# visinf/veto

Hardware: AMD Instinct MI355X
Metric: relation-pairs/sec (PredCls, 36 obj/img) (higher is better)
Workload: dtype fp16 + e4m3 correction terms (fp16 MFMA main product, e4m3 K=128 MFMA cross terms, fp32 accumulate); 1 GPU; BASELINE.json configs[1]: synthetic PredCls, 12 img x 36 obj = 15120 pairs/GPU, d=576, 8 heads, 4 layers, 51 predicates; images_per_gpu=12, objects_per_image=36, pairs_per_gpu=15120, layers=4, heads=8, precision=mixed, parallelism=single GPU

## Files before the change

### veto_amd/csrc/abi_forward.hip

```cpp
#include "abi_internal.h"

namespace {

struct Workspace {
  int32_t *subj, *obj;
  float* lc;
  __bf16* pa;
  float* patch_tab;
  float* x;
  __bf16* a;
  char* big;
  float* xc;
  __bf16* ptab_split;
  float *sw, *ow;
  float* stats;
  __bf16 *ac, *hc;
  size_t total;
};

Workspace carve(char* base, int n_obj, int n_pair, int chunk) {
  Workspace w;
  size_t off = 0;
  auto take = [&](size_t bytes) {
    char* ptr = base ? base + off : nullptr;
    off += align_up(bytes, 256);
    return ptr;
  };
  const size_t prow = (size_t)gemm_rows_padded(n_obj * 16);
  const size_t tile_rows = qkv_attn_rows_padded(chunk);
  const size_t mpad = (size_t)gemm_rows_padded((int)(tile_rows > (size_t)chunk * kTokens ? tile_rows : (size_t)chunk * kTokens));
  const size_t cpad = (size_t)gemm_rows_padded(chunk);
  w.subj = (int32_t*)take((size_t)n_pair * 4);
  w.obj = (int32_t*)take((size_t)n_pair * 4);
  w.lc = (float*)take((size_t)n_obj * 2 * 2 * kDim * 4);
  w.pa = (__bf16*)take(prow * 2 * 2048 * 2);
  w.patch_tab = (float*)take((size_t)n_obj * 16 * 2 * kDim * 4);
  w.x = (float*)take(mpad * kDim * 4);
  w.a = (__bf16*)take(mpad * 2 * kDim * 2);
  {
    const size_t qkv_bytes = mpad * 3 * kDim * 4, fold_bytes = 2 * (align_up(cpad * (size_t)cls_fold_max_heads() * kDim * 4, 256));
    w.big = take(qkv_bytes > fold_bytes ? qkv_bytes : fold_bytes);
  }
  w.xc = (float*)take(cpad * kDim * 4);
  w.ptab_split = (__bf16*)take(prow * 2 * 2 * kDim * 2);
  w.sw = (float*)take(prow * 3 * kDim * 4);
  w.ow = (float*)take(prow * 3 * kDim * 4);
  w.stats = (float*)take(mpad * 2 * 4);
  w.ac = (__bf16*)take(cpad * 2 * kDim * 2);
  w.hc = (__bf16*)take(cpad * 4 * kDim * 2);
  w.total = off;
  return w;
}

struct ForwardPlan {
  int L, H, dhp;
  bool qkv0_tables, fold_last, mixed, fast, mixed_out, cls_mixed, tail_fused, panel, qkv_f24, qa_fused, x_f24;
  bool ffn_ln_next(int l) const { return mixed && panel && l + 1 < L - 1; }
};

ForwardPlan make_plan(veto_handle_t h, bool sat) {
  ForwardPlan p;
  const int L = p.L = h->cfg.layers, H = p.H = h->cfg.heads;
  p.dhp = h->fold_dhp;
  static const bool tables_off = env_knob_is("VETO_QKV0_TABLES", "0");
  p.qkv0_tables = L >= 2 && !tables_off;
  static const bool fold_off = env_knob_is("VETO_CLS_FOLD", "0");
  p.fold_last = !fold_off && H <= cls_fold_max_heads();
  p.mixed = h->cfg.precision != VETO_PRECISE;
  p.fast = h->cfg.precision == VETO_FAST;
  p.mixed_out = p.mixed && attention_reads_tables(H);
  p.cls_mixed = p.mixed;
  static const bool tail_off = env_knob_is("VETO_TAIL_FUSED", "0");
  p.tail_fused = !tail_off && !sat;
  p.panel = !sat;
  static const bool qkv_f24_off = env_knob_is("VETO_QKV_F24", "0");
  p.qkv_f24 = !qkv_f24_off && attention_reads_tables(H);
  static const bool qa_off = env_knob_is("VETO_QKV_ATTN_FUSED", "0");
  p.qa_fused = p.mixed && p.mixed_out && p.tail_fused && !qa_off && qkv_attn_fused_supports(H);
  static const bool x_f24_on = env_knob_is("VETO_X_F24", "1");
  p.x_f24 = x_f24_on && !p.fast && p.mixed && p.mixed_out && p.tail_fused && p.fold_last && p.qkv0_tables && p.qa_fused && L >= 3;
  return p;
}

int object_side(veto_handle_t h, hipStream_t s, const Workspace& ws, const ForwardPlan& p, const veto_inputs_t* in,
                const veto_debug_outputs_t* dbg) {
  const int n_obj = in->n_obj, n_pair = in->n_pair;
  {
    ProfScope ps(h, s, "pair_indices", 0, (double)n_pair * 24);
    HIP_TRY(launch_pair_indices(in->rel_pairs, in->img_obj_offset, in->img_pair_offset, in->n_img, n_pair, ws.subj,
                                ws.obj, dbg ? dbg->subj_inds : nullptr, dbg ? dbg->obj_inds : nullptr, s));
  }
  {
    if (in->bn_batch_stats) HIP_TRY(launch_bn_batch_stats(in->boxes, in->box_mode, n_obj, in->bn_batch_stats, s));
    const ObjPrepArgs a = obj_prep_args(h, in, ws.lc);
    ProfScope ps(h, s, "obj_prep", 2.0 * n_obj * 2 * kDim * (kPosDim + h->cfg.embed_dim), (double)n_obj * 2 * 2 * kDim * 4);
    HIP_TRY(launch_obj_prep(a, s));
  }
  {
// ... 44 lines not shown
    return VETO_OK;
  }

  int qkv0_from_tables() {
    const LayerW& w = h->layers[0];
    const bool mixed = p.mixed;
    if (!attention_reads_tables(p.H)) {
      ProfScope ps(h, s, "qkv0_combine", 0, (double)np * 17 * 3 * kDim * 4 * 3);
      HIP_TRY(launch_qkv0_combine(ws.sw, ws.ow, ws.stats, h->q0_vec, ws.subj + c0, ws.obj + c0, qkv(), np, s));
    }
    for (int t = kTokens - 2; t < kTokens; ++t) {
      if (mixed) HIP_TRY(count_sat(0, VETO_SAT_QKV_IN, ws.a + (size_t)t * 2 * kDim, (long)kTokens * kDim * 4, np, kDim));
      int rc = run_gemm(h, s, "gemm_qkv0_lc", ws.a + (size_t)t * 2 * kDim, mixed ? w.qkv_m : w.qkv, nullptr, nullptr, 0,
                        qkv() + (size_t)t * 3 * kDim, nullptr, (long)kTokens * 3 * kDim, np, 3 * kDim, kDim, EPI_F32, (long)kTokens * 2 * kDim, 0,
                        DropSite(), mixed ? w.exp_m + LIN_QKV : nullptr);
      if (rc) return rc;
    }
    return VETO_OK;
  }

  int attention(int l, bool qkv_f24) {
    const bool last = l == p.L - 1;
    AttnArgs a{};
    a.qkv = qkv(); a.n_pair = np; a.heads = p.H; a.cls_only = last ? 1 : 0;
    a.qkv_f24 = qkv_f24 ? 1 : 0;
    a.o = last ? ws.ac : ws.a;
    a.o_fmt = (!last && p.mixed_out) ? FMT_MIXED : FMT_SPLIT;
    if (l == 0 && p.qkv0_tables && attention_reads_tables(p.H)) {
      a.sw = ws.sw; a.ow = ws.ow; a.stats = ws.stats; a.vec = h->q0_vec; a.subj = ws.subj + c0; a.obj = ws.obj + c0;
    }
    const double nq = last ? 1 : kTokens;
    ProfScope ps(h, s, last ? "attention_cls" : "attention", 4.0 * np * nq * kTokens * kDim,
                 (double)M * 3 * kDim * (qkv_f24 ? 3 : 4) + (double)np * nq * kDim * 4);
    HIP_TRY(launch_attention(a, s));
    if (a.o_fmt == FMT_MIXED) HIP_TRY(count_sat(l, VETO_SAT_ATTN_OUT, ws.a, (long)kDim * 4, M, kDim));
    return VETO_OK;
  }

  int qkv_attention(int l, bool* attn_in_big) {
    const LayerW& w = h->layers[l];
    if (p.qa_fused && l > 0) {
      QkvAttnArgs q{};
      q.a = (const char*)ws.a; q.w = (const char*)w.qkv_m; q.w_exp = w.exp_m + LIN_QKV; q.o = ws.big; q.n_pair = np; q.heads = p.H; q.fast = p.fast ? 1 : 0;
      ProfScope ps(h, s, "qkv_attn_fused", 2.0 * M * 3.0 * kDim * kDim + 4.0 * np * kTokens * kTokens * kDim,
                   (double)M * kDim * 8 + 3.0 * kDim * kDim * 4);
      HIP_TRY(launch_qkv_attn_fused(q, s));
      *attn_in_big = true;
      return VETO_OK;
    }
    const bool mq = p.mixed && l > 0;
    const bool qkv_f24 = mq && p.qkv_f24;
    if (mq) HIP_TRY(count_sat(l, VETO_SAT_QKV_IN, ws.a, (long)kDim * 4, M, kDim));
    int rc = run_gemm(h, s, "gemm_qkv", ws.a, mq ? w.qkv_m : w.qkv, nullptr, nullptr, 0, qkv(), nullptr, 3 * kDim, M, 3 * kDim, kDim,
                      qkv_f24 ? EPI_F24 : EPI_F32, 0, 0, DropSite(), mq ? w.exp_m + LIN_QKV : nullptr);
    return rc ? rc : attention(l, qkv_f24);
  }

  int layer_tail_one_launch(int l, bool attn_in_big) {
    const LayerW& w = h->layers[l];
    const LayerW& nx = h->layers[l + 1];
    const bool ln_next = p.ffn_ln_next(l);
    char* rows = attn_in_big ? ws.big : (char*)ws.a;
    const RowNorm next{ln_next ? nx.ln1_w : nullptr, ln_next ? nx.ln1_b : nullptr, attn_in_big ? ws.a : nullptr};
    FfnArgs f = layer_tail_args(rows, w.mixed(LIN_OUT), RowNorm{w.ln2_w, w.ln2_b, rows}, w.mixed(LIN_FC1), w.mixed(LIN_FC2), ws.x, M, next);
    f.fast = p.fast ? 1 : 0;
    if (p.x_f24) {
// ... 236 lines not shown
```

### veto_amd/csrc/attention.hip

```cpp
#include "common.h"
#include "kernels.h"

#include <cstdio>
#include <cstdlib>
#include <cstring>

namespace veto {

namespace {

constexpr int kWavesPerBlock = 4;

__global__ __launch_bounds__(256) void attention_kernel(AttnArgs a, int dh, int ldh ) {
  extern __shared__ __attribute__((aligned(16))) char smem_raw[];
  const int lane = threadIdx.x & 63, w = threadIdx.x >> 6;
  const long gw = (long)blockIdx.x * kWavesPerBlock + w;
  const int per_wave = 3 * kTokens * ldh + kTokens * 20;
  float* sq = (float*)smem_raw + (size_t)w * per_wave;
  float* sk = sq + kTokens * ldh;
  float* sv = sk + kTokens * ldh;
  float* sp = sv + kTokens * ldh;
  const bool active = gw < (long)a.n_pair * a.heads;
  const int pair = active ? (int)(gw / a.heads) : 0;
  const int head = active ? (int)(gw % a.heads) : 0;
// ... 62 lines not shown
__device__ __forceinline__ void att_split2(float a, float b, uint32_t& hi, uint32_t& lo) {
  uint32_t h, l;
  float l0, l1;
  asm volatile("v_cvt_pk_f16_f32 %0, %1, %2" : "=v"(h) : "v"(a), "v"(b));
  asm("v_fma_mix_f32 %0, %1, -1.0, %2 op_sel_hi:[1,0,0]" : "=v"(l0) : "v"(h), "v"(a));
  asm("v_fma_mix_f32 %0, %1, -1.0, %2 op_sel:[1,0,0] op_sel_hi:[1,0,0]" : "=v"(l1) : "v"(h), "v"(b));
  asm volatile("v_cvt_pk_f16_f32 %0, %1, %2" : "=v"(l) : "v"(l0), "v"(l1));
  hi = h;
  lo = l;
}
typedef _Float16 att_f16x8 __attribute__((ext_vector_type(8)));
__device__ __forceinline__ f32x16 att_mfma(const u32x4& a, const u32x4& b, const f32x16& c) {
  return __builtin_amdgcn_mfma_f32_32x32x16_f16(__builtin_bit_cast(att_f16x8, a), __builtin_bit_cast(att_f16x8, b), c, 0, 0, 0);
}
typedef short att_s16x4 __attribute__((ext_vector_type(4)));
typedef short att_s16x8 __attribute__((ext_vector_type(8)));

template <int V> struct IntTag { static constexpr int value = V; };
template <int I, int N, class F>
__device__ __forceinline__ void att_static_for(F&& f) {
  if constexpr (I < N) {
    f(IntTag<I>());
    att_static_for<I + 1, N>(f);
  }
}
constexpr int kAttWpb = 2;
#ifdef VETO_ATT_STAMPS
__device__ unsigned long long g_att_stamps[8192 * 10];
#define ATT_T(k) do { __builtin_amdgcn_sched_barrier(0); unsigned long long t_; asm volatile("s_memtime %0\n\ts_waitcnt lgkmcnt(0)" : "=s"(t_)::"memory"); \
                      __builtin_amdgcn_sched_barrier(0); att_dt[k] = t_ - att_t; att_t = t_; } while (0)
#else
#define ATT_T(k)
#endif
template <int DH, bool TAB = false, bool F24 = false>
__global__ __launch_bounds__(64 * kAttWpb, TAB && DH > 72 ? 2 : 3) void attention_mfma_kernel(AttnArgs a) {
  static_assert(!(TAB && F24), "the per-object form reads fp32 tables");
  saturating_conversions_on();
#ifdef VETO_ATT_STAMPS
  unsigned long long att_t, att_dt[10] = {0, 0, 0, 0, 0, 0, 0, 0, 0, 0};
  asm volatile("s_memtime %0\n\ts_waitcnt lgkmcnt(0)" : "=s"(att_t)::"memory");
#endif
  constexpr int KS = (DH + 15) / 16;
  constexpr int RB = DH * 2 + (DH % 32 == 0 ? 16 : 0);
  constexpr int NT = (DH + 31) / 32;
  constexpr int QK_PLANE = kTokens * RB;
  constexpr int V_PLANE = (kTokens + 1) * RB;
  constexpr int O_BYTES = kTokens * DH * 4;
  constexpr int PHASE2 = 2 * V_PLANE + O_BYTES;
  constexpr int kConstBytes = TAB ? (3 * DH * 4 + 32 * 4) : 0;
  constexpr int kImgBytes = ((4 * QK_PLANE > PHASE2 ? 4 * QK_PLANE : PHASE2) + 64 + 15) & ~15;
  constexpr int WAVE_LDS = kImgBytes + kConstBytes;
  constexpr int CH = DH / 8;
  constexpr int PER_MAT = kTokens * CH;
  constexpr int ROUNDS = (3 * PER_MAT + 63) / 64;
  static_assert(DH % 8 == 0 && QK_PLANE % 16 == 0 && V_PLANE % 16 == 0, "layout");
  __shared__ __attribute__((aligned(16))) char smem[kAttWpb * WAVE_LDS];

  const int lane = threadIdx.x & 63, w = __builtin_amdgcn_readfirstlane(threadIdx.x >> 6);
  const long item = (long)blockIdx.x * kAttWpb + w;
  if (item >= (long)a.n_pair * a.heads) return;
  char* base = smem + w * WAVE_LDS;
  char* q_hi = base;
  char* q_lo = base + QK_PLANE;
  char* k_hi = base + 2 * QK_PLANE;
  char* k_lo = base + 3 * QK_PLANE;
  char* v_hi = base;
  char* v_lo = v_hi + V_PLANE;

  constexpr int PC = DH / 4;
  constexpr int PER_MAT4 = kTokens * PC;
  constexpr int ROUNDS4 = (3 * PER_MAT4 + 63) / 64;
  f32x4 ld[TAB ? 1 : ROUNDS][2];
  f32x4 lt[TAB ? ROUNDS4 : 1], lo_[TAB ? ROUNDS4 : 1];
  const int pair = (int)(item / a.heads);
  const int head = (int)(item % a.heads);
  const float* src0 = a.qkv + (size_t)pair * kTokens * (3 * kDim) + head * DH;
  const float* tab_s = nullptr;
  const float* tab_o = nullptr;
  if constexpr (TAB) {
    tab_s = a.sw + (size_t)a.subj[pair] * kPatchTokens * (3 * kDim) + head * DH;
    tab_o = a.ow + (size_t)a.obj[pair] * kPatchTokens * (3 * kDim) + head * DH;
  }
  constexpr int kLateFrom = TAB ? (2 * PER_MAT4 + 63) / 64 : ROUNDS;
  constexpr int kRounds = TAB ? ROUNDS4 : ROUNDS;
  float* const c2_lds = (float*)(base + kImgBytes);
  float* const rs_lds = c2_lds + 3 * DH;
  if constexpr (TAB) {
    constexpr int NC2 = 3 * DH / 4;
#pragma unroll
    for (int idx0 = 0; idx0 < NC2; idx0 += 64) {
      const int idx = idx0 + lane;
      if (idx < NC2) {
        const int mat = idx / PC, c4 = idx % PC;
        *(f32x4*)(c2_lds + idx * 4) = *(const f32x4*)(a.vec + head * DH + mat * kDim + c4 * 4);
      }
    }
    if (lane < kTokens) rs_lds[lane] = a.stats[((size_t)pair * kTokens + lane) * 2 + 1];
  }
  auto load_round = [&](auto r_tag) {
    constexpr int r = decltype(r_tag)::value;
    const int e = lane + 64 * r;
    if constexpr (TAB) {
      const int mat = e / PER_MAT4, rem = e % PER_MAT4, i = rem / PC, c4 = rem % PC;
      const bool need = e < 3 * PER_MAT4;
      lo_[r] = f32x4{0.f, 0.f, 0.f, 0.f};
      if (need && i >= 1 && i <= kPatchTokens) {
        const unsigned off = (unsigned)(((i - 1) * (3 * kDim) + mat * kDim + c4 * 4) * 4);
        lo_[r] = *(const f32x4*)((const char*)tab_o + off);
        lt[r] = *(const f32x4*)((const char*)tab_s + off);
      } else if (need) {
        const unsigned off = (unsigned)((mat * kDim + c4 * 4) * 4) + (i == 0 ? 0u : (unsigned)(i * (3 * kDim) * 4));
        const char* src = i == 0 ? (const char*)(a.vec + 2 * (3 * kDim) + head * DH) : (const char*)src0;
        lt[r] = *(const f32x4*)(src + off);
      } else {
        lt[r] = f32x4{0.f, 0.f, 0.f, 0.f};
      }
    } else {
    const int mat = e / PER_MAT, rem = e % PER_MAT, i = rem / CH, c = rem % CH;
    const bool need = e < 3 * PER_MAT && !(a.cls_only && mat == 0 && i > 0);
    if (F24 && need) {
      const char* src = (const char*)a.qkv + (((size_t)pair * kTokens + i) * (3 * kDim) + mat * kDim + head * DH + c * 8) * 3;
      typedef u32x4 u32x4_a8 __attribute__((aligned(8)));
      const u32x4 d01 = *(const u32x4_a8*)src;
      const u32x2 d2 = *(const u32x2*)(src + 16);
      ld[r][0] = f32x4{__uint_as_float(d01[0]), __uint_as_float(d01[1]), __uint_as_float(d01[2]), __uint_as_float(d01[3])};
      ld[r][1] = f32x4{__uint_as_float(d2[0]), __uint_as_float(d2[1]), 0.f, 0.f};
    } else if (need) {
      const unsigned off = (unsigned)((mat * kDim + c * 8) * 4) + (unsigned)(i * (3 * kDim) * 4);
      ld[r][0] = *(const f32x4*)((const char*)src0 + off);
      ld[r][1] = *(const f32x4*)((const char*)src0 + off + 16u);
    } else {
      ld[r][0] = f32x4{0.f, 0.f, 0.f, 0.f};
      ld[r][1] = f32x4{0.f, 0.f, 0.f, 0.f};
    }
    }
  };
  att_static_for<0, kLateFrom>(load_round);
  ATT_T(0);
  auto convert = [&](auto phase_tag) {
    constexpr int PHASE = decltype(phase_tag)::value;
    if constexpr (TAB) {
      att_static_for<0, ROUNDS4>([&](auto r_tag) {
        constexpr int r = decltype(r_tag)::value;
        if constexpr (!(PHASE == 0 ? r >= kLateFrom : 64 * r + 63 < 2 * PER_MAT4)) {
          const int e = lane + 64 * r;
          const int mat = e / PER_MAT4, rem = e % PER_MAT4, i = rem / PC, c4 = rem % PC;
          if (e < 3 * PER_MAT4) {
            if ((PHASE == 0 ? r < kLateFrom : r >= kLateFrom) && i >= 1 && i <= kPatchTokens)
              lt[r] = rs_lds[i] * (lt[r] + lo_[r]) + *(const f32x4*)(c2_lds + mat * DH + c4 * 4);
            if (PHASE == 0 ? mat < 2 : mat == 2) {
              uint32_t h0, l0, h1, l1;
              att_split2(lt[r][0], lt[r][1], h0, l0);
              att_split2(lt[r][2], lt[r][3], h1, l1);
              char* dst = (PHASE == 0 ? (mat == 0 ? q_hi : k_hi) : v_hi) + i * RB + c4 * 8;
              *(u32x2*)dst = u32x2{h0, h1};
              *(u32x2*)(dst + (PHASE == 0 ? QK_PLANE : V_PLANE)) = u32x2{l0, l1};
            }
          }
        }
      });
    } else {
#pragma unroll
    for (int r = 0; r < ROUNDS; ++r) {
      if (PHASE == 0 ? 64 * r >= 2 * PER_MAT : 64 * r + 63 < 2 * PER_MAT) continue;
      const int e = lane + 64 * r;
      if (e >= 3 * PER_MAT) continue;
      const int mat = e / PER_MAT, rem = e % PER_MAT, i = rem / CH, c = rem % CH;
      if (PHASE == 0 ? mat == 2 : mat < 2) continue;
      f32x4 v0 = ld[r][0], v1 = ld[r][1];
      if constexpr (F24) {
        v0 = unpack_f24x4(__float_as_uint(ld[r][0][0]), __float_as_uint(ld[r][0][1]), __float_as_uint(ld[r][0][2]));
        v1 = unpack_f24x4(__float_as_uint(ld[r][0][3]), __float_as_uint(ld[r][1][0]), __float_as_uint(ld[r][1][1]));
      }
      uint32_t h4[4], l4[4];
      att_split2(v0[0], v0[1], h4[0], l4[0]);
      att_split2(v0[2], v0[3], h4[1], l4[1]);
      att_split2(v1[0], v1[1], h4[2], l4[2]);
      att_split2(v1[2], v1[3], h4[3], l4[3]);
      const u32x4 hi = {h4[0], h4[1], h4[2], h4[3]}, lo = {l4[0], l4[1], l4[2], l4[3]};
      if (PHASE == 0) {
// ... 124 lines not shown
    if (e >= nq * CH) continue;
    const int i = e / CH, c = e % CH;
    const f32x4 v0 = *(const f32x4*)(o_lds + i * DH + c * 8);
    const f32x4 v1 = *(const f32x4*)(o_lds + i * DH + c * 8 + 4);
    const size_t row = a.cls_only ? (size_t)pair : (size_t)pair * kTokens + i;
    if (a.o_fmt == FMT_MIXED) {
      store_act8_mixed<true>(a.o + row * (2 * kDim), head * DH + c * 8, v0, v1);
      continue;
    }
    bf16x8 hi, lo;
#pragma unroll
    for (int t = 0; t < 4; ++t) {
      __bf16 hh, ll;
      split_bf16(v0[t], hh, ll);
      hi[t] = hh;
      lo[t] = ll;
      split_bf16(v1[t], hh, ll);
      hi[4 + t] = hh;
      lo[4 + t] = ll;
    }
    __bf16* dst = a.o + row * (2 * kDim) + split_index(head * DH + c * 8);
    *(bf16x8*)dst = hi;
    *(bf16x8*)(dst + 32) = lo;
  }
#ifdef VETO_ATT_STAMPS
  ATT_T(9);
  if (lane == 0) {
    unsigned long long* slot = g_att_stamps + (size_t)(item & 8191) * 10;
    for (int k = 0; k < 10; ++k) slot[k] = att_dt[k];
  }
#endif
}


template <int CTRL>
__device__ __forceinline__ float dpp_rot16(float v) {
  return __int_as_float(__builtin_amdgcn_update_dpp(0, __float_as_int(v), CTRL, 0xF, 0xF, false));
}
__device__ __forceinline__ float row16_sum(float v) {
  v += dpp_rot16<0x128>(v);
  v += dpp_rot16<0x124>(v);
  v += dpp_rot16<0x122>(v);
  v += dpp_rot16<0x121>(v);
  return v;
}

constexpr int kFoldMaxHeads = 12;

__global__ __launch_bounds__(256) void cls_fold_attention_kernel(const float* __restrict__ x, const float* __restrict__ ln_w,
                                                                 const float* __restrict__ ln_b, const float* __restrict__ u,
                                                                 __bf16* __restrict__ abar, int n_pair, int heads, float scale) {
  __shared__ __attribute__((aligned(16))) float a_s[kTokens * kDim];
  __shared__ float s_row[kFoldMaxHeads][4][kTokens];
  __shared__ float p_s[kFoldMaxHeads][kTokens + 1];
  const int pair = blockIdx.x, tid = threadIdx.x, lane = tid & 63, w = tid >> 6;
  if (pair >= n_pair) return;
  {
    const int q = tid & 15;
    const float* xp = x + (size_t)pair * kTokens * kDim;
    for (int j = tid >> 4; j < kTokens; j += 16) {
      f32x4 v[9];
      float sm = 0.f;
#pragma unroll
      for (int i = 0; i < 9; ++i) {
        v[i] = *(const f32x4*)(xp + (size_t)j * kDim + 4 * (q + 16 * i));
        sm += (v[i][0] + v[i][1]) + (v[i][2] + v[i][3]);
// ... 334 lines not shown
}

hipError_t launch_cls_fold_attention(const float* x, const float* ln_w, const float* ln_b, const float* u, __bf16* abar, int n_pair, int heads,
                                     hipStream_t s, bool u_f24) {
  if (heads <= 0 || heads > kFoldMaxHeads || kDim % heads != 0 || n_pair <= 0) return hipErrorInvalidValue;
  const float scale = 1.0f / sqrtf((float)(kDim / heads));
  static const bool valu = env_knob_is("VETO_CLS_MFMA", "0");
  if (u_f24 && valu) return hipErrorInvalidValue;
  if (valu) VETO_LAUNCH(cls_fold_attention_kernel, dim3(n_pair), dim3(256), 0, s, x, ln_w, ln_b, u, abar, n_pair, heads, scale);
  else if (u_f24) VETO_LAUNCH(cls_fold_attention_mfma_kernel<true>, dim3(n_pair), dim3(256), 0, s, x, ln_w, ln_b, u, abar, n_pair, heads, scale);
  else VETO_LAUNCH(cls_fold_attention_mfma_kernel<false>, dim3(n_pair), dim3(256), 0, s, x, ln_w, ln_b, u, abar, n_pair, heads, scale);
#ifdef VETO_CLS_STAMPS
  {
    static int printed = 0;
    if (printed++ == 3) {
      unsigned long long hst[16];
      hipDeviceSynchronize();
      hipMemcpyFromSymbol(hst, HIP_SYMBOL(g_cls_stamps), sizeof(hst));
      fprintf(stderr, "[cls stamps]");
      for (int k = 1; k <= 12; ++k) fprintf(stderr, " %lld", (long long)(hst[k] - hst[k - 1]));
      fprintf(stderr, "  (request | zero | loads->LN start.. | LN+images | barrier | scores | barrier | softmax | barrier | abar | barrier | staging | stores)\n");
    }
  }
#endif
  return hipGetLastError();
}

bool attention_reads_tables(int heads) {
  if (heads <= 0 || kDim % heads != 0) return false;
  const int dh = kDim / heads;
  return dh == 72 || dh == 96;
}

hipError_t launch_attention(const AttnArgs& a, hipStream_t s) {
  if (kDim % a.heads != 0) return hipErrorInvalidValue;
  const int dh = kDim / a.heads;
  if (dh == 72 || dh == 96) {
    const long items = (long)a.n_pair * a.heads;
    unsigned blocks = (unsigned)((items + kAttWpb - 1) / kAttWpb);
    if (a.sw) {
      if (!a.ow || !a.stats || !a.vec || !a.subj || !a.obj || a.cls_only) return hipErrorInvalidValue;
      if (dh == 72) VETO_LAUNCH((attention_mfma_kernel<72, true>), dim3(blocks), dim3(64 * kAttWpb), 0, s, a);
      else VETO_LAUNCH((attention_mfma_kernel<96, true>), dim3(blocks), dim3(64 * kAttWpb), 0, s, a);
#ifdef VETO_ATT_STAMPS
      {
        static unsigned long long all[8192 * 10];
        unsigned long long host[10] = {0};
        hipDeviceSynchronize();
        hipMemcpyFromSymbol(all, HIP_SYMBOL(g_att_stamps), sizeof(all));
        const long nslots = items < 8192 ? items : 8192;
        for (long i = 0; i < nslots; ++i)
          for (int k = 0; k < 10; ++k) host[k] += all[i * 10 + k];
        const double n = (double)nslots;
        static const char* names[10] = {"issue of the early gathers", "wait for the early gathers", "table arithmetic + Q / K conversion", "issue of the late gathers",
                                        "S^T", "softmax", "wait for the late gathers", "V arithmetic + conversion", "P V + staging", "output conversion + stores"};
        double tot = 0;
        for (int k = 0; k < 10; ++k) tot += host[k] / n;
        fprintf(stderr, "[attention stamps, table form, dh %d, last %.0f items] mean shader-clock cycles per item (s_memtime) and share:\n", dh, n);
        for (int k = 0; k < 10; ++k) fprintf(stderr, "    %-38s %8.1f  %5.1f %%\n", names[k], host[k] / n, 100.0 * host[k] / n / tot);
        fprintf(stderr, "    %-38s %8.1f\n", "sum", tot);
      }
#endif
    } else if (a.qkv_f24) {
      if (dh == 72) VETO_LAUNCH((attention_mfma_kernel<72, false, true>), dim3(blocks), dim3(64 * kAttWpb), 0, s, a);
      else VETO_LAUNCH((attention_mfma_kernel<96, false, true>), dim3(blocks), dim3(64 * kAttWpb), 0, s, a);
    } else if (dh == 72) VETO_LAUNCH(attention_mfma_kernel<72>, dim3(blocks), dim3(64 * kAttWpb), 0, s, a);
    else VETO_LAUNCH(attention_mfma_kernel<96>, dim3(blocks), dim3(64 * kAttWpb), 0, s, a);
    return hipGetLastError();
  }
  if (a.sw || a.qkv_f24) return hipErrorInvalidValue;
  if (dh % 4 != 0) return hipErrorInvalidValue;
  const int ldh = dh + 4;
  const size_t lds = (size_t)kWavesPerBlock * (3 * kTokens * ldh + kTokens * 20) * sizeof(float);
  if (lds > 160 * 1024) return hipErrorInvalidValue;
// ... 15 lines not shown
```

### veto_amd/csrc/kernels.h

```cpp
#pragma once
#include "common.h"

namespace veto {

enum Epi { EPI_F32 = 0, EPI_RESID = 1, EPI_GELU_SPLIT = 2, EPI_ATOMIC = 3, EPI_RESID_DROP = 4, EPI_F24 = 5, EPI_SPLIT = 6, EPI_PRE_GELU = 7, EPI_GELU_BWD = 8 };

struct GemmArgs {
  const __bf16* a;
  const __bf16* w;
  const float* bias;
  const float* resid;
  float* c;
  __bf16* c_split;
  int M, N, K;
  long lda;
  long ldr;
  long ldc;
  long ldc_f32;
  float* col_partial;
  int k_splits;
  unsigned long long drop_seed;
  unsigned drop_thresh;
  float drop_scale;
  int tiles_m, tiles_n;
// ... 50 lines not shown
hipError_t launch_mixed_weight_rows(const float* src, __bf16* dst, size_t rows, int K, int* exp_out, hipStream_t s);
hipError_t launch_transpose_split(const float* src, long ld, int M, int N, __bf16* dst, int Mp, hipStream_t s);
hipError_t launch_build_patch_weight(const float* wd, const float* bd, const float* wv, const float* bv,
                                     __bf16* dst, float* bias_cat, hipStream_t s);
hipError_t launch_transpose_pair_proj(const float* src, float* dst, int kin, hipStream_t s);
hipError_t launch_transpose_head(const float* src, float* dst, int n_out, hipStream_t s);

struct ObjPrepArgs {
  const float* boxes;
  int box_mode;
  const int64_t* labels;
  const float* obj_logits;
  const float* embed;
  int num_obj_cls, embed_dim;
  const float* bn_w; const float* bn_b; const float* bn_mean; const float* bn_var;
  const float* pos_w; const float* pos_b;
  const float* loc_wt; const float* loc_b;
  const float* cls_wt; const float* cls_b;
  float* lc;
  float* pos_out;
  int n_obj;
  unsigned long long drop_seed;
  unsigned drop_thresh;
  float drop_scale;
};
hipError_t launch_obj_prep(const ObjPrepArgs& a, hipStream_t s);
hipError_t launch_bn_batch_stats(const float* boxes, int box_mode, int n_obj, float* out, hipStream_t s);
hipError_t launch_patchify(const float* depth, const float* rgb, __bf16* dst, int n_obj, hipStream_t s);

hipError_t launch_pair_indices(const int64_t* rel_pairs, const int32_t* img_obj_off,
                               const int32_t* img_pair_off, int n_img, int n_pair, int32_t* subj,
                               int32_t* obj, int64_t* subj64, int64_t* obj64, hipStream_t s);
hipError_t launch_enumerate_pairs(int n, int64_t* out, hipStream_t s);

struct AssembleArgs {
  const float* patch_tab;
  const float* lc;
  const float* cls_token;
  const float* pos_embedding;
  const float* ln_w; const float* ln_b;
  const int32_t* subj; const int32_t* obj;
  float* x;
  __bf16* a;
  float* stats;
  int a_fmt;
  int x_f24;
  int n_pair;
  unsigned long long drop_seed;
  unsigned drop_thresh;
  float drop_scale;
};
hipError_t launch_assemble(const AssembleArgs& a, hipStream_t s);
hipError_t launch_centre_split(const float* patch_tab, __bf16* dst, int rows, hipStream_t s);
hipError_t launch_qkv0_combine(const float* sw, const float* ow, const float* stats, const float* vec, const int32_t* subj,
                               const int32_t* obj, float* qkv, int n_pair, hipStream_t s);
hipError_t launch_qkv0_consts(const float* wq, const float* gamma, const float* beta, const float* pos, const float* cls, float* wp,
                              float* vec, hipStream_t s);
hipError_t launch_dropout_apply(const float* x, float* y, size_t rows, int n_cols, unsigned long long seed, unsigned thresh,
                                float scale, hipStream_t s);

hipError_t launch_count_saturation(const void* base, long stride_bytes, int rows, int K, unsigned long long* counters, hipStream_t s);
hipError_t launch_layernorm(const float* x, long ldx, const float* w, const float* b, __bf16* dst, int rows,
                            hipStream_t s, int fmt = FMT_SPLIT, long ldd = 0, bool x_f24 = false);
hipError_t launch_unpack_f24(const void* src, float* dst, size_t n, hipStream_t s);

struct AttnArgs {
  const float* qkv;
  __bf16* o;
  int n_pair, heads, cls_only;
  int qkv_f24 = 0;
  int o_fmt = FMT_SPLIT;
  const float* sw = nullptr;
  const float* ow = nullptr;
  const float* stats = nullptr;
  const float* vec = nullptr;
  const int32_t* subj = nullptr;
  const int32_t* obj = nullptr;
};
hipError_t launch_attention(const AttnArgs& a, hipStream_t s);
bool attention_reads_tables(int heads);

struct QkvAttnArgs {
  const char* a;
  const char* w;
  const int* w_exp;
  char* o;
  int n_pair, heads;
  int fast;
};
bool qkv_attn_fused_supports(int heads);
size_t qkv_attn_rows_padded(int n_pair);
hipError_t launch_qkv_attn_fused(const QkvAttnArgs& g, hipStream_t s);
int cls_fold_max_heads();
hipError_t launch_cls_fold_attention(const float* x, const float* ln_w, const float* ln_b, const float* u, __bf16* abar, int n_pair, int heads,
                                     hipStream_t s, bool u_f24 = false);
bool cls_fold_reads_f24();

hipError_t launch_head(const float* cls, const float* wt, const float* bias, float* out, int n_pair,
                       int n_out, hipStream_t s, long ld = kDim);

struct PostArgs {
  const float* rel_logits;
  const float* obj_logits;
  const int64_t* rel_pairs;
  const int32_t* img_obj_off;
  const int32_t* img_pair_off;
  int n_img, n_obj, n_pair, n_rel_cls, n_obj_cls;
  float* obj_scores;
  int64_t* obj_pred;
  float* out_prob;
  int64_t* out_pairs;
  int64_t* out_labels;
  float* out_triple;
// ... 326 lines not shown
```

### veto_amd/csrc/rowops.hip

```cpp
#include "common.h"
#include "kernels.h"

namespace veto {

namespace {

__global__ void split_rows_kernel(const float* __restrict__ src, __bf16* __restrict__ dst, size_t n, int K) {
  size_t i = (size_t)blockIdx.x * blockDim.x + threadIdx.x;
  const size_t stride = (size_t)gridDim.x * blockDim.x;
  for (; i < n; i += stride) {
    const size_t row = i / K;
    const int k = (int)(i % K);
    __bf16 h, l;
    split_bf16(src[i], h, l);
    __bf16* d = dst + row * (2 * (size_t)K) + split_index(k);
    d[0] = h;
    d[32] = l;
  }
}

__global__ void mixed_act_rows_kernel(const float* __restrict__ src, __bf16* __restrict__ dst, size_t n, int K) {
  saturating_conversions_on();
  for (size_t i = ((size_t)blockIdx.x * blockDim.x + threadIdx.x) * 4; i < n; i += (size_t)gridDim.x * blockDim.x * 4) {
    const size_t row = i / K;
// ... 255 lines not shown
#pragma unroll
  for (int y = 0; y < 8; ++y) {
    f32x4 lo, hi;
#pragma unroll
    for (int x = 0; x < 8; ++x) {
      const int row = n * 16 + (y >> 1) * 4 + (x >> 1);
      const int col = mod * 1024 + ((y & 1) * 2 + (x & 1)) * 256 + c;
      const float v = dpa[(size_t)row * ld + col];
      if (x < 4) lo[x] = v; else hi[x - 4] = v;
    }
    *(f32x4*)(out + y * 8) = lo;
    *(f32x4*)(out + y * 8 + 4) = hi;
  }
}

__global__ void pair_indices_kernel(const int64_t* __restrict__ rel_pairs,
                                    const int32_t* __restrict__ img_obj_off,
                                    const int32_t* __restrict__ img_pair_off, int n_img, int n_pair,
                                    int32_t* __restrict__ subj, int32_t* __restrict__ obj,
                                    int64_t* __restrict__ subj64, int64_t* __restrict__ obj64) {
  const int p = blockIdx.x * blockDim.x + threadIdx.x;
  if (p >= n_pair) return;
  int lo = 0, hi = n_img - 1;
  while (lo < hi) {
    const int mid = (lo + hi + 1) >> 1;
    if (img_pair_off[mid] <= p) lo = mid; else hi = mid - 1;
  }
  const int64_t off = img_obj_off[lo];
  const int64_t s = rel_pairs[2 * (size_t)p] + off, o = rel_pairs[2 * (size_t)p + 1] + off;
  subj[p] = (int32_t)s;
  obj[p] = (int32_t)o;
  if (subj64) subj64[p] = s;
  if (obj64) obj64[p] = o;
}

__global__ void enumerate_pairs_kernel(int n, int64_t* __restrict__ out) {
  const long total = n > 1 ? (long)n * (n - 1) : 1;
  const long p = (long)blockIdx.x * blockDim.x + threadIdx.x;
  if (p >= total) return;
  if (n <= 1) { out[0] = 0; out[1] = 0; return; }
  const long i = p / (n - 1), r = p % (n - 1);
  out[2 * p] = i;
  out[2 * p + 1] = r + (r >= i ? 1 : 0);
}

struct RowQ { f32x4 v[9]; };

__device__ __forceinline__ float group16_sum(float v) {
#pragma unroll
  for (int o = 8; o > 0; o >>= 1) v += __shfl_xor(v, o, 64);
  return v;
}

__device__ __forceinline__ void rowq_stats(const RowQ& r, float& mean, float& rstd) {
  float s = 0.f;
#pragma unroll
  for (int j = 0; j < 9; ++j) s += (r.v[j][0] + r.v[j][1]) + (r.v[j][2] + r.v[j][3]);
  mean = group16_sum(s) * (1.f / kDim);
  float sq = 0.f;
#pragma unroll
  for (int j = 0; j < 9; ++j)
#pragma unroll
    for (int e = 0; e < 4; ++e) { const float d = r.v[j][e] - mean; sq += d * d; }
  rstd = 1.f / sqrtf(group16_sum(sq) * (1.f / kDim) + 1e-5f);
}

// ... 321 lines not shown

hipError_t launch_dropout_apply(const float* x, float* y, size_t rows, int n_cols, unsigned long long seed, unsigned thresh,
                                float scale, hipStream_t s) {
  const size_t n = rows * (size_t)n_cols;
  const int blocks = (int)((n + 255) / 256 < 16384 ? (n + 255) / 256 : 16384);
  VETO_LAUNCH(dropout_apply_kernel, dim3(blocks), dim3(256), 0, s, x, y, n, seed, thresh, scale);
  return hipGetLastError();
}

hipError_t launch_bn_batch_stats(const float* boxes, int box_mode, int n_obj, float* out, hipStream_t s) {
  VETO_LAUNCH(bn_batch_stats_kernel, dim3(1), dim3(256), 0, s, boxes, box_mode, n_obj, out);
  return hipGetLastError();
}

hipError_t launch_obj_prep(const ObjPrepArgs& a, hipStream_t s) {
  if (a.num_obj_cls > 256 || a.embed_dim > 256) return hipErrorInvalidValue;
  VETO_LAUNCH(obj_prep_kernel, dim3(a.n_obj, (2 * kDim + 255) / 256), dim3(256), 0, s, a);
  return hipGetLastError();
}

hipError_t launch_patchify(const float* depth, const float* rgb, __bf16* dst, int n_obj, hipStream_t s) {
  VETO_LAUNCH(patchify_kernel, dim3(n_obj, 2), dim3(256), 0, s, depth, rgb, dst);
  return hipGetLastError();
}

hipError_t launch_pair_indices(const int64_t* rel_pairs, const int32_t* img_obj_off,
                               const int32_t* img_pair_off, int n_img, int n_pair, int32_t* subj,
                               int32_t* obj, int64_t* subj64, int64_t* obj64, hipStream_t s) {
  VETO_LAUNCH(pair_indices_kernel, dim3((n_pair + 255) / 256), dim3(256), 0, s, rel_pairs,
                     img_obj_off, img_pair_off, n_img, n_pair, subj, obj, subj64, obj64);
  return hipGetLastError();
}

hipError_t launch_enumerate_pairs(int n, int64_t* out, hipStream_t s) {
  const long total = n > 1 ? (long)n * (n - 1) : 1;
  VETO_LAUNCH(enumerate_pairs_kernel, dim3((unsigned)((total + 255) / 256)), dim3(256), 0, s, n, out);
  return hipGetLastError();
}

hipError_t launch_assemble(const AssembleArgs& a, hipStream_t s) {
  const long blocks = ((long)a.n_pair * kTokens + 15) / 16;
  if (a.stats) {
    VETO_LAUNCH(assemble_kernel<true>, dim3((unsigned)((blocks + 7) / 8 * 8)), dim3(256), 0, s, a);
    for (int t = kPatchTokens + 1; t < kTokens; ++t) {
      const float* xt = a.x_f24 ? (const float*)((const char*)a.x + (size_t)t * kDim * 3) : a.x + (size_t)t * kDim;
      hipError_t e = launch_layernorm(xt, (long)kTokens * kDim, a.ln_w, a.ln_b, a.a + (size_t)t * 2 * kDim, a.n_pair, s,
                                      a.a_fmt == FMT_MIXED ? FMT_MIXED : FMT_SPLIT, (long)kTokens * 2 * kDim, a.x_f24 != 0);
      if (e != hipSuccess) return e;
    }
  } else {
    if (a.x_f24) return hipErrorInvalidValue;
    VETO_LAUNCH(assemble_kernel<false>, dim3((unsigned)((blocks + 7) / 8 * 8)), dim3(256), 0, s, a);
  }
  return hipGetLastError();
}

hipError_t launch_unpack_f24(const void* src, float* dst, size_t n, hipStream_t s) {
  if (n % 4 != 0) return hipErrorInvalidValue;
  const size_t n4 = n / 4;
  const int blocks = (int)((n4 + 255) / 256 < 4096 ? (n4 + 255) / 256 : 4096);
  VETO_LAUNCH(unpack_f24_kernel, dim3(blocks), dim3(256), 0, s, (const char*)src, dst, n4);
  return hipGetLastError();
}

hipError_t launch_qkv0_combine(const float* sw, const float* ow, const float* stats, const float* vec, const int32_t* subj,
                               const int32_t* obj, float* qkv, int n_pair, hipStream_t s) {
// ... 104 lines not shown
```

Before: 1.392 million pairs/s.

## Share subject-table staging across runs of pairs in layer-0 attention

Adds a pass that splits the pair list into runs of consecutive pairs sharing the same subject, chopped into chunks of up to 16. A new attention kernel stages the subject's per-object K/Q/V table rows and the constant vectors into LDS once per run and head, and its waves then process each pair in the run reading the shared copy. The point is to cut repeated global loads of the subject table and per-wave constant staging. A device-side flag turns off the old per-pair kernel when runs are dense enough. The cost is an extra single-block scan launch, larger LDS use that may lower occupancy, and two attention launches where one of them exits early.

```diff
diff --git a/veto_amd/csrc/abi_forward.hip b/veto_amd/csrc/abi_forward.hip
--- a/veto_amd/csrc/abi_forward.hip
+++ b/veto_amd/csrc/abi_forward.hip
@@ -14,6 +14,7 @@
   __bf16* ptab_split;
   float *sw, *ow;
   float* stats;
+  int32_t* runs;
   __bf16 *ac, *hc;
   size_t total;
 };
@@ -46,6 +47,7 @@
   w.sw = (float*)take(prow * 3 * kDim * 4);
   w.ow = (float*)take(prow * 3 * kDim * 4);
   w.stats = (float*)take(mpad * 2 * 4);
+  w.runs = (int32_t*)take(pair_runs_ints(chunk) * 4);
   w.ac = (__bf16*)take(cpad * 2 * kDim * 2);
   w.hc = (__bf16*)take(cpad * 4 * kDim * 2);
   w.total = off;
@@ -54,7 +56,7 @@
 
 struct ForwardPlan {
   int L, H, dhp;
-  bool qkv0_tables, fold_last, mixed, fast, mixed_out, cls_mixed, tail_fused, panel, qkv_f24, qa_fused, x_f24;
+  bool qkv0_tables, att_runs, fold_last, mixed, fast, mixed_out, cls_mixed, tail_fused, panel, qkv_f24, qa_fused, x_f24;
   bool ffn_ln_next(int l) const { return mixed && panel && l + 1 < L - 1; }
 };
 
@@ -64,6 +66,8 @@
   p.dhp = h->fold_dhp;
   static const bool tables_off = env_knob_is("VETO_QKV0_TABLES", "0");
   p.qkv0_tables = L >= 2 && !tables_off;
+  static const bool runs_on = env_knob_is("VETO_ATT_RUNS", "1");
+  p.att_runs = p.qkv0_tables && attention_has_run_form(H) && runs_on;
   static const bool fold_off = env_knob_is("VETO_CLS_FOLD", "0");
   p.fold_last = !fold_off && H <= cls_fold_max_heads();
   p.mixed = h->cfg.precision != VETO_PRECISE;
@@ -174,6 +178,10 @@
     const double nq = last ? 1 : kTokens;
     ProfScope ps(h, s, last ? "attention_cls" : "attention", 4.0 * np * nq * kTokens * kDim,
                  (double)M * 3 * kDim * (qkv_f24 ? 3 : 4) + (double)np * nq * kDim * 4);
+    if (a.sw && p.att_runs) {
+      HIP_TRY(launch_pair_runs(a.subj, np, ws.runs, s));
+      a.runs = ws.runs;
+    }
     HIP_TRY(launch_attention(a, s));
     if (a.o_fmt == FMT_MIXED) HIP_TRY(count_sat(l, VETO_SAT_ATTN_OUT, ws.a, (long)kDim * 4, M, kDim));
     return VETO_OK;
diff --git a/veto_amd/csrc/attention.hip b/veto_amd/csrc/attention.hip
--- a/veto_amd/csrc/attention.hip
+++ b/veto_amd/csrc/attention.hip
@@ -118,34 +118,42 @@
 #else
 #define ATT_T(k)
 #endif
-template <int DH, bool TAB = false, bool F24 = false>
-__global__ __launch_bounds__(64 * kAttWpb, TAB && DH > 72 ? 2 : 3) void attention_mfma_kernel(AttnArgs a) {
+template <int DH, bool TAB, bool RUN>
+struct AttLayout {
+  static constexpr int RB = DH * 2 + (DH % 32 == 0 ? 16 : 0);
+  static constexpr int QK_PLANE = kTokens * RB;
+  static constexpr int V_PLANE = (kTokens + 1) * RB;
+  static constexpr int O_BYTES = kTokens * DH * 4;
+  static constexpr int PHASE2 = 2 * V_PLANE + O_BYTES;
+  static constexpr int kConstBytes = TAB ? ((RUN ? 0 : 3 * DH * 4) + 32 * 4) : 0;
+  static constexpr int kImgBytes = ((4 * QK_PLANE > PHASE2 ? 4 * QK_PLANE : PHASE2) + 64 + 15) & ~15;
+  static constexpr int WAVE_LDS = kImgBytes + kConstBytes;
+  static constexpr int kStageFloats = RUN ? (kPatchTokens * 3 * DH + 3 * DH + 3 * DH) : 0;
+  static constexpr int kStageBytes = kStageFloats * 4;
+};
+
+template <int DH, bool TAB, bool F24, bool RUN>
+__device__ __forceinline__ void attention_item(const AttnArgs& a, const int pair, const int head, char* const base, const int lane,
+                                               const float* const stage) {
   static_assert(!(TAB && F24), "the per-object form reads fp32 tables");
-  saturating_conversions_on();
+  static_assert(TAB || !RUN, "the run form is a form of the per-object one");
 #ifdef VETO_ATT_STAMPS
+  const long item = (long)pair * a.heads + head;
   unsigned long long att_t, att_dt[10] = {0, 0, 0, 0, 0, 0, 0, 0, 0, 0};
   asm volatile("s_memtime %0\n\ts_waitcnt lgkmcnt(0)" : "=s"(att_t)::"memory");
 #endif
+  using Lay = AttLayout<DH, TAB, RUN>;
   constexpr int KS = (DH + 15) / 16;
-  constexpr int RB = DH * 2 + (DH % 32 == 0 ? 16 : 0);
+  constexpr int RB = Lay::RB;
   constexpr int NT = (DH + 31) / 32;
-  constexpr int QK_PLANE = kTokens * RB;
-  constexpr int V_PLANE = (kTokens + 1) * RB;
-  constexpr int O_BYTES = kTokens * DH * 4;
-  constexpr int PHASE2 = 2 * V_PLANE + O_BYTES;
-  constexpr int kConstBytes = TAB ? (3 * DH * 4 + 32 * 4) : 0;
-  constexpr int kImgBytes = ((4 * QK_PLANE > PHASE2 ? 4 * QK_PLANE : PHASE2) + 64 + 15) & ~15;
-  constexpr int WAVE_LDS = kImgBytes + kConstBytes;
+  constexpr int QK_PLANE = Lay::QK_PLANE;
+  constexpr int V_PLANE = Lay::V_PLANE;
+  constexpr int kImgBytes = Lay::kImgBytes;
   constexpr int CH = DH / 8;
   constexpr int PER_MAT = kTokens * CH;
   constexpr int ROUNDS = (3 * PER_MAT + 63) / 64;
   static_assert(DH % 8 == 0 && QK_PLANE % 16 == 0 && V_PLANE % 16 == 0, "layout");
-  __shared__ __attribute__((aligned(16))) char smem[kAttWpb * WAVE_LDS];
-
-  const int lane = threadIdx.x & 63, w = __builtin_amdgcn_readfirstlane(threadIdx.x >> 6);
-  const long item = (long)blockIdx.x * kAttWpb + w;
-  if (item >= (long)a.n_pair * a.heads) return;
-  char* base = smem + w * WAVE_LDS;
+
   char* q_hi = base;
   char* q_lo = base + QK_PLANE;
   char* k_hi = base + 2 * QK_PLANE;
@@ -157,28 +165,29 @@
   constexpr int PER_MAT4 = kTokens * PC;
   constexpr int ROUNDS4 = (3 * PER_MAT4 + 63) / 64;
   f32x4 ld[TAB ? 1 : ROUNDS][2];
-  f32x4 lt[TAB ? ROUNDS4 : 1], lo_[TAB ? ROUNDS4 : 1];
-  const int pair = (int)(item / a.heads);
-  const int head = (int)(item % a.heads);
+  f32x4 lt[TAB ? ROUNDS4 : 1], lo_[TAB && !RUN ? ROUNDS4 : 1];
   const float* src0 = a.qkv + (size_t)pair * kTokens * (3 * kDim) + head * DH;
   const float* tab_s = nullptr;
   const float* tab_o = nullptr;
   if constexpr (TAB) {
-    tab_s = a.sw + (size_t)a.subj[pair] * kPatchTokens * (3 * kDim) + head * DH;
+    if constexpr (!RUN) tab_s = a.sw + (size_t)a.subj[pair] * kPatchTokens * (3 * kDim) + head * DH;
     tab_o = a.ow + (size_t)a.obj[pair] * kPatchTokens * (3 * kDim) + head * DH;
   }
   constexpr int kLateFrom = TAB ? (2 * PER_MAT4 + 63) / 64 : ROUNDS;
   constexpr int kRounds = TAB ? ROUNDS4 : ROUNDS;
-  float* const c2_lds = (float*)(base + kImgBytes);
-  float* const rs_lds = c2_lds + 3 * DH;
-  if constexpr (TAB) {
+  const float* const c2_lds = RUN ? stage + kPatchTokens * 3 * DH : (const float*)(base + kImgBytes);
+  const float* const cls_lds = c2_lds + 3 * DH;
+  float* const rs_lds = (float*)(base + kImgBytes) + (RUN ? 0 : 3 * DH);
+  if constexpr (TAB && RUN) {
+    if (lane < kTokens) rs_lds[lane] = a.stats[((size_t)pair * kTokens + lane) * 2 + 1];
+  } else if constexpr (TAB) {
     constexpr int NC2 = 3 * DH / 4;
 #pragma unroll
     for (int idx0 = 0; idx0 < NC2; idx0 += 64) {
       const int idx = idx0 + lane;
       if (idx < NC2) {
         const int mat = idx / PC, c4 = idx % PC;
-        *(f32x4*)(c2_lds + idx * 4) = *(const f32x4*)(a.vec + head * DH + mat * kDim + c4 * 4);
+        *(f32x4*)(base + kImgBytes + idx * 16) = *(const f32x4*)(a.vec + head * DH + mat * kDim + c4 * 4);
       }
     }
     if (lane < kTokens) rs_lds[lane] = a.stats[((size_t)pair * kTokens + lane) * 2 + 1];
@@ -189,6 +198,18 @@
     if constexpr (TAB) {
       const int mat = e / PER_MAT4, rem = e % PER_MAT4, i = rem / PC, c4 = rem % PC;
       const bool need = e < 3 * PER_MAT4;
+      if constexpr (RUN) {
+        if (need && i >= 1 && i <= kPatchTokens) {
+          const unsigned off = (unsigned)(((i - 1) * (3 * kDim) + mat * kDim + c4 * 4) * 4);
+          lt[r] = *(const f32x4*)((const char*)tab_o + off);
+        } else if (need && i > kPatchTokens) {
+          const unsigned off = (unsigned)((mat * kDim + c4 * 4) * 4) + (unsigned)(i * (3 * kDim) * 4);
+          lt[r] = *(const f32x4*)((const char*)src0 + off);
+        } else {
+          lt[r] = f32x4{0.f, 0.f, 0.f, 0.f};
+        }
+        return;
+      }
       lo_[r] = f32x4{0.f, 0.f, 0.f, 0.f};
       if (need && i >= 1 && i <= kPatchTokens) {
         const unsigned off = (unsigned)(((i - 1) * (3 * kDim) + mat * kDim + c4 * 4) * 4);
@@ -232,6 +253,12 @@
           const int e = lane + 64 * r;
           const int mat = e / PER_MAT4, rem = e % PER_MAT4, i = rem / PC, c4 = rem % PC;
           if (e < 3 * PER_MAT4) {
+            if constexpr (RUN) {
+              if ((PHASE == 0 ? r < kLateFrom : r >= kLateFrom) && i >= 1 && i <= kPatchTokens)
+                lt[r] = rs_lds[i] * (*(const f32x4*)(stage + ((i - 1) * 3 + mat) * DH + c4 * 4) + lt[r]) + *(const f32x4*)(c2_lds + mat * DH + c4 * 4);
+              else if ((PHASE == 0 ? r < kLateFrom : r >= kLateFrom) && i == 0)
+                lt[r] = *(const f32x4*)(cls_lds + mat * DH + c4 * 4);
+            } else
             if ((PHASE == 0 ? r < kLateFrom : r >= kLateFrom) && i >= 1 && i <= kPatchTokens)
               lt[r] = rs_lds[i] * (lt[r] + lo_[r]) + *(const f32x4*)(c2_lds + mat * DH + c4 * 4);
             if (PHASE == 0 ? mat < 2 : mat == 2) {
@@ -422,6 +449,59 @@
 #endif
 }
 
+template <int DH, bool TAB = false, bool F24 = false>
+__global__ __launch_bounds__(64 * kAttWpb, TAB && DH > 72 ? 2 : 3) void attention_mfma_kernel(AttnArgs a) {
+  saturating_conversions_on();
+  __shared__ __attribute__((aligned(16))) char smem[kAttWpb * AttLayout<DH, TAB, false>::WAVE_LDS];
+  if constexpr (TAB) {
+    if (a.runs && a.runs[1] != 0) return;
+  }
+  const int lane = threadIdx.x & 63, w = __builtin_amdgcn_readfirstlane(threadIdx.x >> 6);
+  const long item = (long)blockIdx.x * kAttWpb + w;
+  if (item >= (long)a.n_pair * a.heads) return;
+  attention_item<DH, TAB, F24, false>(a, (int)(item / a.heads), (int)(item % a.heads), smem + w * AttLayout<DH, TAB, false>::WAVE_LDS, lane, nullptr);
+}
+
+template <int DH> constexpr int kAttRunWaves = 4;
+template <int DH>
+__global__ __launch_bounds__(64 * kAttRunWaves<DH>, 2) void attention_runs_kernel(AttnArgs a) {
+  saturating_conversions_on();
+  using Lay = AttLayout<DH, true, true>;
+  constexpr int W = kAttRunWaves<DH>;
+  __shared__ __attribute__((aligned(16))) char smem[Lay::kStageBytes + W * Lay::WAVE_LDS];
+  static_assert(Lay::kStageBytes % 16 == 0 && sizeof(smem) <= 160 * 1024, "layout");
+  if (a.runs[1] == 0) return;
+  const int head = blockIdx.x % a.heads, n_runs = a.runs[0];
+  float* const stage = (float*)smem;
+  const int lane = threadIdx.x & 63, w = __builtin_amdgcn_readfirstlane(threadIdx.x >> 6);
+  char* const base = smem + Lay::kStageBytes + w * Lay::WAVE_LDS;
+#pragma unroll 1
+  for (int sr = blockIdx.x / a.heads; sr < n_runs; sr += gridDim.x / a.heads) {
+    const int first = a.runs[2 + sr], end = min(a.runs[3 + sr], a.n_pair);
+    if (first < 0 || first >= end) continue;
+    const int len = end - first;
+    {
+      constexpr int PC = DH / 4, NSW = kPatchTokens * 3 * PC, NALL = NSW + 6 * PC;
+      const float* tab_s = a.sw + (size_t)a.subj[first] * kPatchTokens * (3 * kDim) + head * DH;
+      const float* vec = a.vec + head * DH;
+#pragma unroll
+      for (int idx0 = 0; idx0 < NALL; idx0 += 64 * W) {
+        const int idx = idx0 + (int)threadIdx.x;
+        if (idx < NALL) {
+          const int row = idx / PC, c4 = idx % PC;
+          const float* src = row < kPatchTokens * 3 ? tab_s + (row / 3) * (3 * kDim) + (row % 3) * kDim
+                                                    : vec + (row - kPatchTokens * 3 >= 3 ? 2 * (3 * kDim) + (row - kPatchTokens * 3 - 3) * kDim
+                                                                                         : (row - kPatchTokens * 3) * kDim);
+          *(f32x4*)(stage + idx * 4) = *(const f32x4*)(src + c4 * 4);
+        }
+      }
+    }
+    __syncthreads();
+#pragma unroll 1
+    for (int k = w; k < len; k += W) attention_item<DH, true, false, true>(a, first + k, head, base, lane, stage);
+    __syncthreads();
+  }
+}
 
 template <int CTRL>
 __device__ __forceinline__ float dpp_rot16(float v) {
@@ -822,6 +902,8 @@
   return dh == 72 || dh == 96;
 }
 
+bool attention_has_run_form(int heads) { return heads > 0 && kDim % heads == 0 && kDim / heads == 72; }
+
 hipError_t launch_attention(const AttnArgs& a, hipStream_t s) {
   if (kDim % a.heads != 0) return hipErrorInvalidValue;
   const int dh = kDim / a.heads;
@@ -830,6 +912,13 @@
     unsigned blocks = (unsigned)((items + kAttWpb - 1) / kAttWpb);
     if (a.sw) {
       if (!a.ow || !a.stats || !a.vec || !a.subj || !a.obj || a.cls_only) return hipErrorInvalidValue;
+      if (a.runs && a.n_pair >= 2) {
+        const unsigned rblocks = (unsigned)((long)((a.n_pair + kAttRun - 1) / kAttRun) * a.heads);
+        if (dh != 72) return hipErrorInvalidValue;
+        VETO_LAUNCH(attention_runs_kernel<72>, dim3(rblocks), dim3(64 * kAttRunWaves<72>), 0, s, a);
+        const hipError_t e = hipGetLastError();
+        if (e != hipSuccess) return e;
+      }
       if (dh == 72) VETO_LAUNCH((attention_mfma_kernel<72, true>), dim3(blocks), dim3(64 * kAttWpb), 0, s, a);
       else VETO_LAUNCH((attention_mfma_kernel<96, true>), dim3(blocks), dim3(64 * kAttWpb), 0, s, a);
 #ifdef VETO_ATT_STAMPS
diff --git a/veto_amd/csrc/kernels.h b/veto_amd/csrc/kernels.h
--- a/veto_amd/csrc/kernels.h
+++ b/veto_amd/csrc/kernels.h
@@ -106,6 +106,12 @@
                                const int32_t* img_pair_off, int n_img, int n_pair, int32_t* subj,
                                int32_t* obj, int64_t* subj64, int64_t* obj64, hipStream_t s);
 hipError_t launch_enumerate_pairs(int n, int64_t* out, hipStream_t s);
+#ifndef VETO_ATT_RUN
+#define VETO_ATT_RUN 16
+#endif
+constexpr int kAttRun = VETO_ATT_RUN;
+inline size_t pair_runs_ints(int n_pair) { return (size_t)n_pair + 3; }
+hipError_t launch_pair_runs(const int32_t* subj, int n_pair, int32_t* runs, hipStream_t s);
 
 struct AssembleArgs {
   const float* patch_tab;
@@ -150,9 +156,11 @@
   const float* vec = nullptr;
   const int32_t* subj = nullptr;
   const int32_t* obj = nullptr;
+  const int32_t* runs = nullptr;
 };
 hipError_t launch_attention(const AttnArgs& a, hipStream_t s);
 bool attention_reads_tables(int heads);
+bool attention_has_run_form(int heads);
 
 struct QkvAttnArgs {
   const char* a;
diff --git a/veto_amd/csrc/rowops.hip b/veto_amd/csrc/rowops.hip
--- a/veto_amd/csrc/rowops.hip
+++ b/veto_amd/csrc/rowops.hip
@@ -311,6 +311,72 @@
   obj[p] = (int32_t)o;
   if (subj64) subj64[p] = s;
   if (obj64) obj64[p] = o;
+}
+
+constexpr int kRunThreads = 1024, kRunPer = 16;
+__global__ __launch_bounds__(kRunThreads) void pair_runs_kernel(const int32_t* __restrict__ subj, int n_pair, int32_t* __restrict__ runs) {
+  __shared__ int w_max[kRunThreads / 64], w_sum[kRunThreads / 64];
+  const int tid = threadIdx.x, lane = tid & 63, w = tid >> 6;
+  int count = 0;
+  for (int tile0 = 0; tile0 < n_pair; tile0 += kRunThreads * kRunPer) {
+    const int p0 = tile0 + tid * kRunPer;
+    int sv[kRunPer];
+#pragma unroll
+    for (int j = 0; j < kRunPer; ++j) sv[j] = p0 + j < n_pair ? subj[p0 + j] : -1;
+    const int prev = (tid > 0 && p0 - 1 < n_pair) ? subj[p0 - 1] : -1;
+    unsigned opens = 0;
+    int last_open = -1;
+#pragma unroll
+    for (int j = 0; j < kRunPer; ++j) {
+      if (p0 + j < n_pair && sv[j] != (j ? sv[j - 1] : prev)) {
+        opens |= 1u << j;
+        last_open = p0 + j;
+      }
+    }
+    int v = last_open;
+#pragma unroll
+    for (int o = 1; o < 64; o <<= 1) {
+      const int t = __shfl_up(v, o, 64);
+      if (lane >= o) v = max(v, t);
+    }
+    if (lane == 63) w_max[w] = v;
+    __syncthreads();
+    int run0 = __shfl_up(v, 1, 64);
+    if (lane == 0) run0 = -1;
+    for (int k = 0; k < w; ++k) run0 = max(run0, w_max[k]);
+    unsigned starts = 0;
+    int n_start = 0;
+#pragma unroll
+    for (int j = 0; j < kRunPer; ++j) {
+      if (opens >> j & 1) run0 = p0 + j;
+      if (p0 + j < n_pair && (p0 + j - run0) % kAttRun == 0) {
+        starts |= 1u << j;
+        ++n_start;
+      }
+    }
+    v = n_start;
+#pragma unroll
+    for (int o = 1; o < 64; o <<= 1) {
+      const int t = __shfl_up(v, o, 64);
+      if (lane >= o) v += t;
+    }
+    if (lane == 63) w_sum[w] = v;
+    __syncthreads();
+    int at = count + v - n_start;
+    for (int k = 0; k < kRunThreads / 64; ++k) {
+      if (k < w) at += w_sum[k];
+      count += w_sum[k];
+    }
+#pragma unroll
+    for (int j = 0; j < kRunPer; ++j)
+      if (starts >> j & 1) runs[2 + at++] = p0 + j;
+    __syncthreads();
+  }
+  if (tid == 0) {
+    runs[0] = count;
+    runs[1] = 2 * count <= n_pair ? 1 : 0;
+    runs[2 + count] = n_pair;
+  }
 }
 
 __global__ void enumerate_pairs_kernel(int n, int64_t* __restrict__ out) {
@@ -698,6 +764,12 @@
   return hipGetLastError();
 }
 
+hipError_t launch_pair_runs(const int32_t* subj, int n_pair, int32_t* runs, hipStream_t s) {
+  if (!subj || !runs || n_pair <= 0) return hipErrorInvalidValue;
+  VETO_LAUNCH(pair_runs_kernel, dim3(1), dim3(kRunThreads), 0, s, subj, n_pair, runs);
+  return hipGetLastError();
+}
+
 hipError_t launch_enumerate_pairs(int n, int64_t* out, hipStream_t s) {
   const long total = n > 1 ? (long)n * (n - 1) : 1;
   VETO_LAUNCH(enumerate_pairs_kernel, dim3((unsigned)((total + 255) / 256)), dim3(256), 0, s, n, out);
```

After: 1.392 million pairs/s, median of 2. About the same (+0.0%).
